# liubingqi7/audio-motion-avatar

Hardware: AMD Instinct MI355X
Metric: rendered frames/sec @512x512, 10k Gaussians (static triplane decode + SMPL-X LBS + tile rasterize) (higher is better)
Workload: dtype f32 (LBS blend-shape product: fp16 x 2 split operands with fp32 accumulation, fp32-equivalent; everything else plain fp32)

## Files before the change

### audio-motion-avatar_amd/_lib.py

```python
import ctypes
import os

_HERE = os.path.dirname(os.path.abspath(__file__))
LIB_PATH = os.environ.get("AMAV_LIB") or os.path.join(_HERE, "csrc", "libamav_hip.so")

c_float_p = ctypes.c_void_p


class AmavError(RuntimeError):
    pass


class Attr(ctypes.Structure):

    _fields_ = [("ptr", ctypes.c_void_p), ("frame_stride", ctypes.c_int64), ("elem_stride", ctypes.c_int32),
                ("_pad", ctypes.c_int32)]


class RasterArgs(ctypes.Structure):
    _fields_ = [
        ("num_frames", ctypes.c_int32), ("num_gaussians", ctypes.c_int32), ("height", ctypes.c_int32),
        ("width", ctypes.c_int32),
        ("means3d", Attr), ("rotations", Attr), ("scales", Attr), ("opacities", Attr), ("colors", Attr),
        ("viewmatrix", ctypes.c_void_p), ("projmatrix", ctypes.c_void_p), ("tanfov", ctypes.c_void_p),
# ... 81 lines not shown
    "amav_gemm_library_version": (ctypes.c_char_p, []),
    "amav_last_error": (ctypes.c_char_p, []),
    "amav_device_count": (ctypes.c_int, []),
    "amav_event_create": (ctypes.c_int, [ctypes.POINTER(ctypes.c_void_p)]),
    "amav_event_destroy": (ctypes.c_int, [ctypes.c_void_p]),
    "amav_event_record": (ctypes.c_int, [ctypes.c_void_p, ctypes.c_void_p]),
    "amav_event_elapsed_ms": (ctypes.c_int, [ctypes.c_void_p, ctypes.c_void_p, ctypes.POINTER(ctypes.c_float)]),
    "amav_camera_from_intrinsics": (ctypes.c_int, [ctypes.c_int, c_float_p, c_float_p, ctypes.c_int, ctypes.c_int,
                                                   ctypes.c_float, ctypes.c_float, c_float_p, c_float_p, c_float_p,
                                                   c_float_p, ctypes.c_void_p]),
    "amav_rasterize_workspace_bytes": (ctypes.c_size_t, [ctypes.c_int, ctypes.c_int, ctypes.c_int, ctypes.c_int,
                                                         ctypes.c_int64]),
    "amav_rasterize_forward": (ctypes.c_int, [ctypes.POINTER(RasterArgs), ctypes.c_void_p]),
    "amav_rasterize_decode_forward": (ctypes.c_int, [ctypes.POINTER(RasterArgs), ctypes.POINTER(DecodeSource),
                                                     ctypes.c_void_p]),
    "amav_rasterize_status": (ctypes.c_int, [ctypes.c_void_p, ctypes.POINTER(ctypes.c_int64),
                                             ctypes.POINTER(ctypes.c_int64), ctypes.POINTER(ctypes.c_int32),
                                             ctypes.c_void_p]),
    "amav_rasterize_backward_bytes": (ctypes.c_size_t, [ctypes.c_int, ctypes.c_int, ctypes.c_int64]),
    "amav_rasterize_backward": (ctypes.c_int, [ctypes.POINTER(RasterArgs), ctypes.POINTER(RasterBackwardArgs),
                                               ctypes.c_void_p]),
    "amav_frames_to_rgb8": (ctypes.c_int, [ctypes.c_int64, c_float_p, ctypes.c_void_p, ctypes.c_void_p]),
    "amav_add_layernorm": (ctypes.c_int, [ctypes.c_int64, ctypes.c_int, ctypes.c_int64, c_float_p, c_float_p, c_float_p,
                                          c_float_p, c_float_p, c_float_p, c_float_p, ctypes.c_float, c_float_p,
                                          ctypes.c_void_p, ctypes.c_int, ctypes.c_int, ctypes.c_void_p]),
    "amav_geglu": (ctypes.c_int, [ctypes.c_int64, ctypes.c_int, c_float_p, ctypes.c_int64, c_float_p, c_float_p,
                                  ctypes.c_void_p, ctypes.c_int, ctypes.c_void_p]),
    "amav_split_operand": (ctypes.c_int, [ctypes.c_int64, ctypes.c_int, c_float_p, ctypes.c_int64, ctypes.c_int,
                                          ctypes.c_int, ctypes.c_int, ctypes.c_void_p, ctypes.c_void_p]),
    "amav_frames_wire_bytes": (ctypes.c_size_t, [ctypes.c_int, ctypes.c_int, ctypes.c_int, ctypes.c_int64]),
# ... 137 lines not shown
```

### audio-motion-avatar_amd/csrc/amav_common.h

```cpp
#pragma once
#include <hip/hip_runtime.h>

#include <cstdarg>
#include <cstdint>
#include <cstdio>

#include "../../include/amav.h"

namespace amav {

constexpr int kWave = 64;

char *error_buffer();

inline int fail(int code, const char *fmt, ...) {
    va_list ap;
    va_start(ap, fmt);
    vsnprintf(error_buffer(), 512, fmt, ap);
    va_end(ap);
    return code;
}

#define AMAV_REQUIRE(cond, ...)                                         \
    do {                                                                \
// ... 3 lines not shown
inline int check_launch(const char *what) {
    hipError_t e = hipGetLastError();
    if (e != hipSuccess) return fail(AMAV_ERR_LAUNCH, "%s: %s", what, hipGetErrorString(e));
    return AMAV_OK;
}

inline size_t align_up(size_t v, size_t a) { return (v + a - 1) / a * a; }

constexpr int kWireHeaderInts = 16;
constexpr int kWireMagic = 0x414d4156;
constexpr int kWireTileBytes = 16 * 16 * 3;
inline size_t wire_payload_at(int F, int tiles) { return ((size_t)(kWireHeaderInts + F + tiles) * 4 + 15) / 16 * 16; }

int option_attn();
int option_lbs();

hipError_t zero_async(void *ptr, size_t bytes, hipStream_t stream);

struct Carver {
    char *base;
    size_t off = 0;
    explicit Carver(void *b) : base(static_cast<char *>(b)) {}
    template <typename T>
    T *take(size_t count) {
        off = align_up(off, 256);
        T *p = base ? reinterpret_cast<T *>(base + off) : nullptr;
        off += count * sizeof(T);
        return p;
    }
    size_t total() const { return align_up(off, 256); }
// ... 4 lines not shown
```

### audio-motion-avatar_amd/csrc/api.hip

```cpp
#include <atomic>
#include <cstdlib>
#include <cstring>

#include "amav_common.h"

namespace amav {

char *error_buffer() {
    static thread_local char buf[512] = {0};
    return buf;
}

static std::atomic<int> g_option_attn{-1}, g_option_lbs{-1};
int option_attn() { return g_option_attn.load(std::memory_order_relaxed); }
int option_lbs() { return g_option_lbs.load(std::memory_order_relaxed); }

static int clear_mode() {
    static const int mode = [] {
        const char *e = getenv("AMAV_CLEAR");
        return (e && e[0] == 'm') ? 1 : 0;
    }();
    return mode;
}

__global__ __launch_bounds__(256) void zero_words_kernel(unsigned *__restrict__ dst, size_t words) {
    const size_t i = (size_t)blockIdx.x * 256 + threadIdx.x;
    const size_t quads = words >> 2;
    if ((reinterpret_cast<uintptr_t>(dst) & 15) == 0) {
        if (i < quads) reinterpret_cast<uint4 *>(dst)[i] = make_uint4(0u, 0u, 0u, 0u);
        if (i < (words & 3)) dst[quads * 4 + i] = 0u;
// ... 104 lines not shown
extern "C" int amav_set_option(const char *name, const char *value) {
    AMAV_REQUIRE(name && value, "amav_set_option: NULL argument");
    const bool dflt = strcmp(value, "default") == 0;
    if (strcmp(name, "attn") == 0) {
        const int v = dflt ? -1 : strcmp(value, "f32") == 0 ? 0 : strcmp(value, "bf16") == 0 ? 1 : strcmp(value, "fp16") == 0 ? 2 : -2;
        AMAV_REQUIRE(v != -2, "amav_set_option: attn = \"%s\" (expected fp16, bf16, f32 or default)", value);
        amav::g_option_attn.store(v);
        return AMAV_OK;
    }
    if (strcmp(name, "lbs") == 0) {
        const int v = dflt ? -1 : strcmp(value, "f32") == 0 ? 0 : strcmp(value, "split") == 0 ? 1 : -2;
        AMAV_REQUIRE(v != -2, "amav_set_option: lbs = \"%s\" (expected split, f32 or default)", value);
        amav::g_option_lbs.store(v);
        return AMAV_OK;
    }
    return amav::fail(AMAV_ERR_INVALID_ARG, "amav_set_option: unknown option \"%s\"", name);
}
```

### audio-motion-avatar_amd/csrc/decode_quad.h

```cpp
#pragma once
#include <hip/hip_runtime.h>

namespace amav {
namespace decode {

template <int K>
__device__ __forceinline__ float quad_bcast(float v) {
    return __int_as_float(__builtin_amdgcn_mov_dpp(__float_as_int(v), K * 0x55, 0xf, 0xf, true));
}
template <int K>
__device__ __forceinline__ int quad_bcast_i(int v) {
    return __builtin_amdgcn_mov_dpp(v, K * 0x55, 0xf, 0xf, true);
}

__device__ __forceinline__ void quad_point(float v0, float v1, float v2, float &p0, float &p1, float &p2) {
#pragma clang fp contract(off)
    p0 = fmaf(quad_bcast<0>(v0) + quad_bcast<1>(v0), 0.5f, (quad_bcast<2>(v0) + quad_bcast<3>(v0)) * 0.5f) * 0.5f;
    p1 = fmaf(quad_bcast<0>(v1) + quad_bcast<1>(v1), 0.5f, (quad_bcast<2>(v1) + quad_bcast<3>(v1)) * 0.5f) * 0.5f;
    p2 = ((quad_bcast<0>(v2) + quad_bcast<1>(v2)) * 0.5f + (quad_bcast<2>(v2) + quad_bcast<3>(v2)) * 0.5f) * 0.5f;
}

__device__ __forceinline__ float clamp_unit(float p, float radius) {
#pragma clang fp contract(off)
    return fminf(fmaxf(p / radius, -1.0f), 1.0f);
}

struct PlaneTaps {
    int ix0, iy0;
    float wx0, wx1, wy0, wy1;
    int off[4];
    float w[4];
    bool in[4];
};
__device__ __forceinline__ PlaneTaps plane_taps(float gx, float gy, int R) {
#pragma clang fp contract(off)
    const float sx = fmaf(gx + 1.0f, (float)R, -1.0f), sy = fmaf(gy + 1.0f, (float)R, -1.0f);
    const float fx = floorf(sx * 0.5f), fy = floorf(sy * 0.5f);
    PlaneTaps t;
    t.ix0 = (int)fx, t.iy0 = (int)fy;
    t.wx1 = fmaf(sx, 0.5f, -fx), t.wx0 = fmaf(-sx, 0.5f, fx + 1.0f);
    t.wy1 = fmaf(sy, 0.5f, -fy), t.wy0 = fmaf(-sy, 0.5f, fy + 1.0f);
#pragma unroll
    for (int dy = 0; dy < 2; ++dy)
#pragma unroll
        for (int dx = 0; dx < 2; ++dx) {
            const int x = t.ix0 + dx, y = t.iy0 + dy;
            const bool in = x >= 0 && x < R && y >= 0 && y < R;
            const int cx = min(max(x, 0), R - 1), cy = min(max(y, 0), R - 1);
            t.in[dy * 2 + dx] = in;
            t.w[dy * 2 + dx] = in ? (dx ? t.wx1 : t.wx0) * (dy ? t.wy1 : t.wy0) : 0.0f;
            t.off[dy * 2 + dx] = (cy * R + cx) * 4;
        }
    return t;
}

struct QuadTaps {
    int off[12];
    float w[12];
};
__device__ __forceinline__ QuadTaps quad_taps(float p0, float p1, float p2, float radius, int R, int q) {
#pragma clang fp contract(off)
    const float u0 = clamp_unit(p0, radius), u1 = clamp_unit(p1, radius), u2 = clamp_unit(p2, radius);
    const PlaneTaps pt = plane_taps(q == 2 ? u1 : u0, q == 0 ? u1 : u2, R);
    QuadTaps t;
    const int RR4 = R * R * 4;
#pragma unroll
    for (int k = 0; k < 4; ++k) {
        t.w[k] = quad_bcast<0>(pt.w[k]), t.w[4 + k] = quad_bcast<1>(pt.w[k]), t.w[8 + k] = quad_bcast<2>(pt.w[k]);
        t.off[k] = quad_bcast_i<0>(pt.off[k]);
        t.off[4 + k] = RR4 + quad_bcast_i<1>(pt.off[k]);
        t.off[8 + k] = 2 * RR4 + quad_bcast_i<2>(pt.off[k]);
    }
    return t;
}

__device__ __forceinline__ float4 group_raw(const float4 (&tv)[12], const float (&tw)[12], const float4 (&wp)[4],
                                            float p0, float p1, float p2) {
#pragma clang fp contract(off)
    float4 acc = make_float4(0.f, 0.f, 0.f, 0.f);
#pragma unroll
    for (int k = 0; k < 12; ++k) {
        const float w = tw[k];
        const float4 v = tv[k];
        acc.x = fmaf(v.x, w, acc.x), acc.y = fmaf(v.y, w, acc.y), acc.z = fmaf(v.z, w, acc.z), acc.w = fmaf(v.w, w, acc.w);
    }
    const float4 w0 = wp[0], w1 = wp[1], w2 = wp[2], w3 = wp[3];
    acc.x += fmaf(w0.z, p2, fmaf(w0.y, p1, w0.x * p0)) + w0.w;
    acc.y += fmaf(w1.z, p2, fmaf(w1.x, p0, w1.y * p1)) + w1.w;
// ... 33 lines not shown
```

### audio-motion-avatar_amd/csrc/rasterizer.hip

```cpp
#include <algorithm>
#include <cmath>
#include <cstddef>
#include <cstdlib>

#include "amav_common.h"
#include "decode_quad.h"
#include "raster_project.h"
#include "raster_workspace.h"

namespace amav {
namespace raster {

#ifndef AMAV_BIN_ABLATE
#define AMAV_BIN_ABLATE 0
#endif
#ifndef AMAV_ABLATE
#define AMAV_ABLATE 0
#endif
constexpr int kRenderWavesPerSimd = 4;
constexpr int kFusedMinFrames = 96;
constexpr int kSortCap = 512;
constexpr int kBigLdsCap = 2048;
constexpr int kBigBlocks = 1280;

// ... 17 lines not shown
    float4 *geom;
    uint4 *rectd;
    int *tile_off;
    unsigned long long *keys;
    unsigned *sorted;
    int *big_list;
    int4 *queue;
    int *empty_list;
    int *slice_counts;
    Status *status;
};

static inline int bin_slices(int F) { return F >= kFusedMinFrames ? 0 : std::min(16, std::max(1, (256 + F - 1) / F)); }

static inline size_t queue_capacity(int F, int gx, int gy) { return (size_t)F * ((gy + kQueues - 1) / kQueues) * gx; }

static Buffers carve(void *ws, int F, int N, int gx, int gy, long long cap, size_t *bytes) {
    const int T = gx * gy;
    Carver c(ws);
    Buffers b;
    b.status = c.take<Status>(1);
    b.geom = c.take<float4>(((size_t)F * N + 1024) * 3);
    b.rectd = c.take<uint4>((size_t)F * N + 1024);
    b.tile_off = c.take<int>((size_t)F * (T + 1));
    b.keys = c.take<unsigned long long>((size_t)cap);
    b.sorted = c.take<unsigned>((size_t)cap);
    b.big_list = c.take<int>((size_t)F * T);
    b.queue = c.take<int4>((size_t)kQueues * kBuckets * queue_capacity(F, gx, gy));
    b.empty_list = c.take<int>((size_t)F * T);
    b.slice_counts = c.take<int>((size_t)F * bin_slices(F) * T);
// ... 21 lines not shown
    int wire_cap;
    unsigned wire_bg;
    int stash;
    int slices;
    Buffers buf;
    struct {
        const float4 *proj;
        const float *vertices;
        const int *idx4;
        const float *transl;
        const float4 *wpoint;
        float4 *out;
        float radius;
        int R, V;
        int rec_lds;
    } dec;
};

__device__ __forceinline__ int opaque(int x) {
    asm volatile("" : "+v"(x));
    return x;
}
__device__ __forceinline__ int lane_now() {
    int l;
    asm volatile("v_mbcnt_lo_u32_b32 %0, -1, 0\n\tv_mbcnt_hi_u32_b32 %0, -1, %0" : "=v"(l));
    return l;
}
__device__ __forceinline__ unsigned zero_now() {
    unsigned z;
    asm volatile("v_mov_b32 %0, 0" : "=v"(z));
// ... 178 lines not shown
    for (int o = 32; o > 0; o >>= 1) up += __shfl_xor(up, o, 64);
    if ((threadIdx.x & 63) == 0) part[threadIdx.x >> 6] = up;
    __syncthreads();
    if (threadIdx.x == 0) {
        const int sum = part[0] + part[1] + part[2] + part[3];
        if (sum) atomicAdd(reinterpret_cast<unsigned long long *>(&p.buf.status->total), (unsigned long long)sum);
    }
}

template <bool kFused, bool kPacked, bool kDecode = false>
__global__ __launch_bounds__(1024) void bin_kernel(Params p) {
    extern __shared__ int bin_lds[];
    int *counts = bin_lds;
    int *cursor = bin_lds + p.T;
    int *scratch = bin_lds + 2 * p.T + 3 * kQueues * (kBuckets + 1);
    uint2 *stash = reinterpret_cast<uint2 *>(scratch + 48);
    const int f = blockIdx.x;
#ifdef AMAV_BIN_STAMPS
#define AMAV_BIN_STAMP(k)                                                                                        \
    do {                                                                                                         \
        __syncthreads();                                                                                         \
        if (p.stamps && threadIdx.x == 0) p.stamps[(size_t)p.F * p.T * 6 + (size_t)f * 8 + (k)] = __builtin_amdgcn_s_memrealtime(); \
    } while (0)
#else
#define AMAV_BIN_STAMP(k)
#endif
    AMAV_BIN_STAMP(0);
    for (int t = threadIdx.x; t < p.T; t += blockDim.x) counts[t] = 0;
    if (kDecode && threadIdx.x < 4) scratch[40 + threadIdx.x] = 0;
    __syncthreads();

// ... 9 lines not shown
        auto project = [&](const GaussRec &rec, int i) {
            int up = 0;
            float4 g[3] = {make_float4(0.f, 0.f, 0.f, 0.f), make_float4(0.f, 0.f, 0.f, 0.f), make_float4(0.f, 0.f, 0.f, 0.f)};
            uint4 rd = preprocess_one(p, rec, cam, up, g);
            const bool real = i < p.N;
            if (!real) rd = make_uint4(0u, 0u, 0u, 0u), up = 0;
            upstream += up;
#if AMAV_BIN_ABLATE != 1
            if (rd.w) {
                const int rx0 = rd.x & 0xffff, ry0 = rd.x >> 16, rx1 = rd.y & 0xffff, ry1 = rd.y >> 16;
                for (int ty = ry0; ty < ry1; ++ty)
                    for (int tx = rx0; tx < rx1; ++tx) atomicAdd(&counts[ty * p.gx + tx], 1);
            }
#endif
            if (p.stash && real)
                stash[i] = make_uint2((rd.x & 0xff) | ((rd.x >> 16) << 8) | ((rd.y & 0xff) << 16) | ((rd.y >> 16) << 24), rd.z);
            const size_t gi = real ? (size_t)f * p.N + i : (size_t)p.F * p.N + threadIdx.x;
            if (!kDecode) p.buf.rectd[gi] = rd;
            float4 *dst = p.buf.geom + gi * 3;
            dst[0] = g[0], dst[1] = g[1], dst[2] = g[2];
        };
        if (kDecode) {
            constexpr int kRounds = 4, kSlot = kRounds * 128, kWaves = 8;
            float4 *recs = reinterpret_cast<float4 *>(reinterpret_cast<char *>(bin_lds) + p.dec.rec_lds);
            int *filled = scratch + 40, *drained = scratch + 42;
            const int N = p.N, groups = (N + kSlot - 1) / kSlot;
            bool stuck = false;
            auto wait_ge = [&](int *c, int v) {
                for (int n = 0; __hip_atomic_load(c, __ATOMIC_RELAXED, __HIP_MEMORY_SCOPE_WORKGROUP) < v; ++n) {
                    if (n > (1 << 22)) {
                        stuck = true;
                        break;
                    }
                    __builtin_amdgcn_s_sleep(1);
                }
                __builtin_amdgcn_fence(__ATOMIC_ACQUIRE, "workgroup");
            };
            auto signal = [&](int *c) {
                __builtin_amdgcn_fence(__ATOMIC_RELEASE, "workgroup");
                if ((threadIdx.x & 63) == 0) __hip_atomic_fetch_add(c, 1, __ATOMIC_RELAXED, __HIP_MEMORY_SCOPE_WORKGROUP);
            };
            if (threadIdx.x < kWaves * 64) {
                const int q = threadIdx.x & 3, slot = threadIdx.x >> 2;
                const int R = p.dec.R;
                const float4 *pl0 = p.dec.proj + (size_t)f * 3 * R * R * 4 + q;
                const float *vf = p.dec.vertices + (size_t)f * p.dec.V * 3;
                const float4 wp[4] = {p.dec.wpoint[q * 4], p.dec.wpoint[q * 4 + 1], p.dec.wpoint[q * 4 + 2], p.dec.wpoint[q * 4 + 3]};
                float tx = 0.f, ty = 0.f, tz = 0.f;
                if (p.dec.transl && q == 0) tx = p.dec.transl[f * 3], ty = p.dec.transl[f * 3 + 1], tz = p.dec.transl[f * 3 + 2];
                auto index_of = [&](int n) { return p.dec.idx4[(size_t)min(n, N - 1) * 4 + q]; };
                int idx[kRounds];
                float v[kRounds][3];
#pragma unroll
                for (int r = 0; r < kRounds; ++r) idx[r] = index_of(r * 128 + slot);
#pragma unroll
                for (int r = 0; r < kRounds; ++r) {
                    const float *vp = vf + (size_t)idx[r] * 3;
                    v[r][0] = vp[0], v[r][1] = vp[1], v[r][2] = vp[2];
                }
#pragma unroll
                for (int r = 0; r < kRounds; ++r) idx[r] = index_of(kSlot + r * 128 + slot);
                for (int k = 0; k < groups; ++k) {
                    const int s = k & 1;
                    float4 *ring = recs + s * 4 * kSlot + q * kSlot;
                    wait_ge(&drained[s], kWaves * (k >> 1));
#pragma unroll
                    for (int r = 0; r < kRounds; ++r) {
                        float p0, p1, p2;
                        decode::quad_point(v[r][0], v[r][1], v[r][2], p0, p1, p2);
                        const decode::QuadTaps t = decode::quad_taps(p0, p1, p2, p.dec.radius, R, q);
                        float4 tv[12];
#pragma unroll
                        for (int j = 0; j < 12; ++j) tv[j] = pl0[t.off[j]];
                        ring[r * 128 + slot] = decode::quad_record(tv, t.w, wp, p0, p1, p2, tx, ty, tz, q);
                    }
                    signal(&filled[s]);
#pragma unroll
                    for (int r = 0; r < kRounds; ++r) {
                        const float *vp = vf + (size_t)idx[r] * 3;
                        v[r][0] = vp[0], v[r][1] = vp[1], v[r][2] = vp[2];
                    }
#pragma unroll
                    for (int r = 0; r < kRounds; ++r) idx[r] = index_of((k + 2) * kSlot + r * 128 + slot);
                }
            } else {
                const int j = threadIdx.x - kWaves * 64;
                float4 *outf = p.dec.out + (size_t)f * N * 4;
                for (int k = 0; k < groups; ++k) {
                    const int s = k & 1;
                    const float4 *ring = recs + s * 4 * kSlot + j;
                    wait_ge(&filled[s], kWaves * ((k >> 1) + 1));
                    GaussRec rec;
                    rec.r0 = ring[0], rec.r1 = ring[kSlot], rec.r2 = ring[2 * kSlot], rec.r3 = ring[3 * kSlot];
                    signal(&drained[s]);
                    const int i = k * kSlot + j;
                    if (i < N) {
                        float4 *o = outf + (size_t)i * 4;
                        o[0] = rec.r0, o[1] = rec.r1, o[2] = rec.r2, o[3] = rec.r3;
                    }
// ... 19 lines not shown
        block_exclusive_scan(upstream, scratch, &upstream_total);
        if (threadIdx.x == 0)
            atomicAdd(reinterpret_cast<unsigned long long *>(&p.buf.status->total), (unsigned long long)upstream_total);
    } else {
        int *sc = p.buf.slice_counts + (size_t)f * p.slices * p.T;
        for (int t = threadIdx.x; t < p.T; t += blockDim.x) {
            int run = 0;
            for (int b = 0; b < p.slices; ++b) {
                const int c = sc[(size_t)b * p.T + t];
                sc[(size_t)b * p.T + t] = run;
                run += c;
            }
            counts[t] = run;
        }
    }
    __syncthreads();
    AMAV_BIN_STAMP(1);

    const int per = (p.T + (int)blockDim.x - 1) / (int)blockDim.x;
    const int t0 = threadIdx.x * per;
    int local = 0;
    for (int k = 0; k < per; ++k)
        if (t0 + k < p.T) local += counts[t0 + k];
    int total;
    int run = block_exclusive_scan(local, scratch, &total);
    int *off = p.buf.tile_off + (size_t)f * (p.T + 1);
    for (int k = 0; k < per; ++k) {
        const int t = t0 + k;
        if (t < p.T) {
            const int c = counts[t];
            cursor[t] = run;
            off[t] = run;
            run += c;
            if (c > kSortCap) {
                const int slot = atomicAdd(&p.buf.status->big_count, 1);
                p.buf.big_list[slot] = f * p.T + t;
            }
        }
    }
    const bool fits = (long long)total <= p.cap_per_frame;
// ... 1153 lines not shown
    AMAV_REQUIRE(a->num_frames > 0 && a->num_gaussians > 0 && a->height > 0 && a->width > 0,
                 "amav_rasterize_forward: bad sizes F=%d N=%d H=%d W=%d", a->num_frames, a->num_gaussians, a->height,
                 a->width);
    AMAV_REQUIRE(a->means3d.ptr && a->rotations.ptr && a->scales.ptr && a->opacities.ptr && a->colors.ptr,
                 "amav_rasterize_forward: NULL Gaussian attribute");
    AMAV_REQUIRE(a->viewmatrix && a->projmatrix && a->tanfov, "amav_rasterize_forward: NULL camera");
    AMAV_REQUIRE(a->out_rgba != nullptr, "amav_rasterize_forward: out_rgba is NULL");
    AMAV_REQUIRE(a->workspace != nullptr, "amav_rasterize_forward: workspace is NULL");
    AMAV_REQUIRE(a->instance_capacity >= 0, "amav_rasterize_forward: negative instance_capacity");
    AMAV_REQUIRE((reinterpret_cast<uintptr_t>(a->out_rgba) & 15) == 0, "amav_rasterize_forward: out_rgba not 16-B aligned");
    const int F = a->num_frames, N = a->num_gaussians;
    const int gx = (a->width + kTile - 1) / kTile, gy = (a->height + kTile - 1) / kTile;
    AMAV_REQUIRE(gx < 65536 && gy < 65536, "amav_rasterize_forward: image too large");
    const int T = gx * gy;
    AMAV_REQUIRE((long long)F * T < (1ll << 31), "amav_rasterize_forward: F * tiles overflows int32");
    const size_t bin_lds = ((size_t)2 * T + 48 + 3 * kQueues * (kBuckets + 1)) * sizeof(int);
    AMAV_REQUIRE(bin_lds <= 160 * 1024, "amav_rasterize_forward: %d tiles need %zu B of LDS in the binning block (max 160 KiB)",
                 T, bin_lds);
    const bool stash = bin_lds + 8 + (size_t)N * 8 <= 160 * 1024 && gx <= 255 && gy <= 255 && a->out_radii == nullptr;
    const size_t rec_lds = align_up(bin_lds + (size_t)N * 8, 16);
    const bool fits_decode = stash && rec_lds + 1024 * 64 <= 160 * 1024;
    const long long cap_per_frame = a->instance_capacity / F;
    AMAV_REQUIRE(cap_per_frame < (1ll << 31), "amav_rasterize_forward: per-frame instance capacity overflows int32");
    size_t need = 0;
    Params p;
    p.dec = {};
    p.buf = carve(a->workspace, F, N, gx, gy, cap_per_frame * F, &need);
    if (a->workspace_bytes < need)
        return fail(AMAV_ERR_WORKSPACE, "amav_rasterize_forward: workspace %zu < required %zu", a->workspace_bytes, need);
    p.F = F, p.N = N, p.H = a->height, p.W = a->width, p.gx = gx, p.gy = gy, p.T = T;
    p.means3d = a->means3d, p.rotations = a->rotations, p.scales = a->scales, p.opacities = a->opacities;
    p.colors = a->colors;
    p.view = a->viewmatrix, p.proj = a->projmatrix, p.tanfov = a->tanfov;
    p.bg[0] = a->bg[0], p.bg[1] = a->bg[1], p.bg[2] = a->bg[2];
    p.scale_modifier = a->scale_modifier;
    p.apply_activations = a->apply_activations;
// ... 53 lines not shown
                     "amav_rasterize_decode_forward: bad decode source (R=%d V=%d radius=%g)", d->resolution, d->num_verts,
                     (double)d->radius);
        AMAV_REQUIRE(d->proj && d->vertices && d->idx4 && d->head_w_point,
                     "amav_rasterize_decode_forward: NULL decode input");
        AMAV_REQUIRE(((reinterpret_cast<uintptr_t>(d->proj) | reinterpret_cast<uintptr_t>(d->idx4) |
                       reinterpret_cast<uintptr_t>(d->head_w_point)) & 15) == 0,
                     "amav_rasterize_decode_forward: proj/idx4/head_w_point not 16-B aligned");
        p.dec.proj = reinterpret_cast<const float4 *>(d->proj);
        p.dec.vertices = d->vertices;
        p.dec.idx4 = d->idx4;
        p.dec.transl = d->transl;
        p.dec.wpoint = reinterpret_cast<const float4 *>(d->head_w_point);
        p.dec.out = reinterpret_cast<float4 *>(const_cast<float *>(b0));
        p.dec.radius = d->radius;
        p.dec.R = d->resolution, p.dec.V = d->num_verts;
        p.dec.rec_lds = (int)rec_lds;
        if (!decode_fused) {
            const int rc = amav_triplane_sample_decode_indexed(F, N, d->resolution, d->num_verts, d->proj, d->vertices,
                                                               d->idx4, d->transl, d->radius, d->head_w_point,
                                                               const_cast<float *>(b0), stream);
            if (rc != AMAV_OK) return rc;
        }
    }
    if (zero_async(p.buf.status, sizeof(Status), stream) != hipSuccess)
        return fail(AMAV_ERR_LAUNCH, "amav_rasterize_forward: status clear failed");
    if (p.wire_header && zero_async(p.wire_header, (size_t)kWireHeaderInts * 4, stream) != hipSuccess)
        return fail(AMAV_ERR_LAUNCH, "amav_rasterize_forward: wire header clear failed");

    if (F < kFusedMinFrames && F <= 65535) {
        const dim3 pre_grid((unsigned)((N + 255) / 256), (unsigned)F);
        if (packed)
            preprocess_kernel<true><<<pre_grid, 256, 0, stream>>>(p);
        else
            preprocess_kernel<false><<<pre_grid, 256, 0, stream>>>(p);
        const dim3 slice_grid((unsigned)p.slices, (unsigned)F);
        slice_count_kernel<<<slice_grid, 1024, (size_t)T * sizeof(int), stream>>>(p);
        bin_kernel<false, false><<<F, 1024, bin_lds, stream>>>(p);
        slice_scatter_kernel<<<slice_grid, 1024, (size_t)T * sizeof(int), stream>>>(p);
    } else if (decode_fused)
        bin_kernel<true, true, true><<<F, 1024, rec_lds + 1024 * 64, stream>>>(p);
    else if (packed)
        bin_kernel<true, true><<<F, 1024, bin_lds + (stash ? 8 + (size_t)N * 8 : 0), stream>>>(p);
    else
        bin_kernel<true, false><<<F, 1024, bin_lds + (stash ? 8 + (size_t)N * 8 : 0), stream>>>(p);
    sort_big_kernel<<<kBigBlocks, 256, 0, stream>>>(p);
    const unsigned blocks = render_grid(a->out_inv_depth != nullptr);
    if (a->profile_start_event) (void)hipEventRecord(static_cast<hipEvent_t>(a->profile_start_event), stream);
    if (a->out_inv_depth)
        render_kernel<true><<<blocks, 64, 0, stream>>>(p);
    else
        render_kernel<false><<<blocks, 64, 0, stream>>>(p);
    if (a->profile_stop_event) (void)hipEventRecord(static_cast<hipEvent_t>(a->profile_stop_event), stream);
    return check_launch("amav_rasterize_forward");
}

extern "C" int amav_rasterize_forward(const amav_raster_args *a, void *stream) { return rasterize_forward(a, nullptr, stream); }

extern "C" int amav_rasterize_decode_forward(const amav_raster_args *a, const amav_decode_source *d, void *stream) {
    AMAV_REQUIRE(d != nullptr, "amav_rasterize_decode_forward: decode source is NULL");
    return rasterize_forward(a, d, stream);
}

namespace amav {
namespace raster {
__global__ __launch_bounds__(256) void tile_counts_kernel(int F, int T, const Status *__restrict__ st,
                                                          const int *__restrict__ tile_off, int *__restrict__ out) {
    const int i = blockIdx.x * blockDim.x + threadIdx.x;
    if (i >= F * T) return;
    const int f = i / T, t = i - f * T;
    const int *off = tile_off + (size_t)f * (T + 1);
// ... 45 lines not shown
```

### audio-motion-avatar_amd/csrc/triplane.hip

```cpp
#include <cstdlib>

#include "amav_common.h"
#include "decode_quad.h"
#include "triplane_region.h"

namespace amav {
namespace triplane {

typedef float f32x4 __attribute__((ext_vector_type(4)));

template <int kUnroll, bool kNT>
__global__ __launch_bounds__(256) void project_kernel(int C, int RR, const float *__restrict__ tokens,
                                                      long long frame_stride, const float *__restrict__ wplane,
                                                      float *__restrict__ out, const float *__restrict__ boxes,
                                                      float radius, int R) {
    extern __shared__ __align__(16) float w_lds[];
    const int bx = blockIdx.z;
    int q = bx * blockDim.x + threadIdx.x;
    const int plane = blockIdx.x, f = blockIdx.y;
    if (boxes) {
        const TexelRect rc = region_of(boxes + (size_t)f * 6, plane, radius, R);
        const int c0 = rc.x0 >> 2, per_row = (rc.x1 >> 2) - c0 + 1, rows = rc.y1 - rc.y0 + 1;
        if (bx * (int)blockDim.x >= per_row * rows) return;
        const int row = q / per_row;
// ... 197 lines not shown
        float acc = 0.0f;
#pragma unroll
        for (int q = 0; q < 4; ++q)
            if (off[q] >= 0) acc += img[off[q]] * wt[q];
        tile[k * 65 + lane] = acc;
    }
    __syncthreads();
    for (int p = wave; p < 64; p += 4) {
        if (n0 + p < N) out[((size_t)f * N + n0 + p) * 3 * C + oc0 + lane] = tile[lane * 65 + p];
    }
}

__global__ __launch_bounds__(1024) void bbox_kernel(int N, const float *__restrict__ points, float *__restrict__ boxes) {
    __shared__ float part[16][7];
    const int f = blockIdx.x;
    const float *pp = points + (size_t)f * N * 3;
    const int total = 3 * N;
    float lo[3] = {__builtin_inff(), __builtin_inff(), __builtin_inff()};
    float hi[3] = {-__builtin_inff(), -__builtin_inff(), -__builtin_inff()};
    float bad = 0.f;
    for (int e0 = threadIdx.x * 3; e0 < total; e0 += blockDim.x * 3) {
#pragma unroll
        for (int d = 0; d < 3; ++d) {
            const float v = pp[e0 + d];
            lo[d] = fminf(lo[d], v), hi[d] = fmaxf(hi[d], v);
            if (v != v) bad = 1.f;
        }
    }
#pragma unroll
    for (int o = 32; o > 0; o >>= 1) {
#pragma unroll
        for (int d = 0; d < 3; ++d) {
            lo[d] = fminf(lo[d], __shfl_xor(lo[d], o, 64));
            hi[d] = fmaxf(hi[d], __shfl_xor(hi[d], o, 64));
        }
        bad = fmaxf(bad, __shfl_xor(bad, o, 64));
    }
    const int wave = threadIdx.x >> 6, nwaves = blockDim.x >> 6;
    if ((threadIdx.x & 63) == 0) {
#pragma unroll
        for (int d = 0; d < 3; ++d) part[wave][d] = lo[d], part[wave][3 + d] = hi[d];
        part[wave][6] = bad;
    }
    __syncthreads();
    if (threadIdx.x < 6) {
        const int d = threadIdx.x;
        float any_bad = 0.f, v = part[0][d];
        for (int w = 0; w < nwaves; ++w) {
            any_bad += part[w][6];
            v = d < 3 ? fminf(v, part[w][d]) : fmaxf(v, part[w][d]);
        }
        if (any_bad > 0.f) v = d < 3 ? -__builtin_inff() : __builtin_inff();
        boxes[(size_t)f * 6 + d] = v;
    }
}

}
}

using namespace amav;
using namespace amav::triplane;

extern "C" int amav_points_bbox(int F, int N, const float *points, float *out_boxes, void *stream) {
    AMAV_REQUIRE(F > 0 && N > 0 && points && out_boxes, "amav_points_bbox: bad sizes F=%d N=%d or NULL pointer", F, N);
    bbox_kernel<<<F, 1024, 0, static_cast<hipStream_t>(stream)>>>(N, points, out_boxes);
    return check_launch("amav_points_bbox");
}

extern "C" int amav_triplane_project(int F, int C, int R, const float *tokens, int64_t frame_stride,
// ... 88 lines not shown
```

### audio-motion-avatar_amd/csrc/triplane_region.h

```cpp
#pragma once
#include <hip/hip_runtime.h>

namespace amav {
namespace triplane {

struct TexelRect {
    int x0, x1, y0, y1;
};
__device__ __forceinline__ int tap_floor(float p, float radius, int R) {
    const float u = fminf(fmaxf(p / radius, -1.0f), 1.0f);
    return (int)floorf(((u + 1.0f) * (float)R - 1.0f) * 0.5f);
}
__device__ __forceinline__ TexelRect region_of(const float *__restrict__ box, int plane, float radius, int R) {
    const int ax = plane == 2 ? 1 : 0, ay = plane == 0 ? 1 : 2;
    TexelRect r;
    r.x0 = min(max(tap_floor(box[ax], radius, R), 0), R - 1);
    r.x1 = min(max(tap_floor(box[3 + ax], radius, R) + 1, 0), R - 1);
    r.y0 = min(max(tap_floor(box[ay], radius, R), 0), R - 1);
    r.y1 = min(max(tap_floor(box[3 + ay], radius, R) + 1, 0), R - 1);
    return r;
}

}
}
```

### audio-motion-avatar_amd/ops.py

```python
import ctypes
import os

import torch

from . import _lib
from ._lib import (AmavError, Attr, BodyTables, DecodeSource, LbsBackwardArgs, PoseParts, RasterArgs,
                   RasterBackwardArgs, TriplaneDecodeBackwardArgs, check)

SCALE_BIAS = 3.9
OPACITY_BIAS = 0.0
SCALE_MAX = 0.1
GAUSS_STRIDE = 16
REC_XYZ, REC_OPACITY, REC_ROT, REC_SCALE, REC_COLOR = 0, 3, 4, 8, 12


def tensor_version(t: torch.Tensor) -> int:
    return -1 if t.is_inference() else t._version


def set_option(name: str, value: str):
    check(_lib.lib().amav_set_option(name.encode(), value.encode()), "amav_set_option")


def _stream():
    return ctypes.c_void_p(torch.cuda.current_stream().cuda_stream)


def _need(t: torch.Tensor, name: str, dtype=torch.float32):
    if not isinstance(t, torch.Tensor):
        raise AmavError(f"{name}: expected a torch.Tensor, got {type(t).__name__}")
    if not t.is_cuda:
        raise AmavError(f"{name}: tensor is on {t.device}; this package only runs on an MI355X (HIP) device")
    if t.dtype != dtype:
        raise AmavError(f"{name}: dtype {t.dtype}, expected {dtype}")
    return t

# ... 1373 lines not shown
```

### include/amav.h

```cpp
#ifndef AMAV_H
#define AMAV_H

#include <stddef.h>
#include <stdint.h>

#ifdef __cplusplus
extern "C" {
#endif

#define AMAV_OK 0
#define AMAV_ERR_INVALID_ARG (-1)
#define AMAV_ERR_LAUNCH (-2)
#define AMAV_ERR_WORKSPACE (-3)
#define AMAV_ERR_NO_DEVICE (-4)

#define AMAV_TILE 16
#define AMAV_GAUSS_STRIDE 16

const char *amav_version(void);
const char *amav_last_error(void);
int amav_device_count(void);
int amav_set_option(const char *name, const char *value);

int amav_event_create(void **event);
// ... 61 lines not shown
    float *debug_alpha;
} amav_raster_backward_args;
size_t amav_rasterize_backward_bytes(int num_frames, int num_gaussians, int64_t max_frame_instances);
int amav_rasterize_backward(const amav_raster_args *fwd, const amav_raster_backward_args *bwd, void *stream);

typedef struct amav_decode_source {
    int32_t resolution, num_verts;
    const float *proj;
    const float *vertices;
    const int32_t *idx4;
    const float *transl;
    float radius;
    const float *head_w_point;
} amav_decode_source;
int amav_rasterize_decode_forward(const amav_raster_args *args, const amav_decode_source *src, void *stream);

int amav_frames_to_rgb8(int64_t num_pixels, const float *rgba_dev, uint8_t *out_rgb8_dev, void *stream);

int amav_rasterize_tile_counts(const void *workspace, int num_frames, int num_gaussians, int height, int width,
                               int64_t instance_capacity, int32_t *out_counts_dev, void *stream);
size_t amav_frames_wire_bytes(int num_frames, int height, int width, int64_t capacity_tiles);
int amav_frames_pack_tiles(int num_frames, int height, int width, const float *rgba_dev, const float *background_host3,
                           const int32_t *tile_hint_dev, int64_t capacity_tiles, void *wire_dev, size_t wire_bytes,
                           void *stream);
int amav_frames_unpack_tiles(int num_buffers, int num_frames, int height, int width, int64_t capacity_tiles,
                             const void *wire_all_dev, size_t wire_stride, uint8_t *out_rgb8_dev, int32_t *status_dev,
                             void *stream);
int amav_frames_unpack_tiles_delta(int num_buffers, int num_frames, int height, int width, int64_t capacity_tiles,
                                   const void *wire_all_dev, size_t wire_stride, uint8_t *out_rgb8_dev,
                                   int32_t *tile_state_dev, int32_t *status_dev, void *stream);
// ... 199 lines not shown
```

Baseline: 321,500.

## Stage triplane texel region into LDS for fused decode-bin kernel

In the fused decode+bin kernel, each frame's vertex bounding box is computed in-block and mapped to texel rectangles on the three planes. When those fit in the spare LDS, the rectangles are copied into shared memory and bilinear taps read from LDS instead of global memory. To free LDS, the per-gaussian stash is written to global memory first and reloaded into LDS after binning. This adds a bbox reduction, extra barriers and a full 160 KiB LDS allocation per block, which may cut occupancy, and can be turned off with the decode_taps=global option.

```diff
diff --git a/audio-motion-avatar_amd/_lib.py b/audio-motion-avatar_amd/_lib.py
--- a/audio-motion-avatar_amd/_lib.py
+++ b/audio-motion-avatar_amd/_lib.py
@@ -119,6 +119,7 @@
     "amav_rasterize_forward": (ctypes.c_int, [ctypes.POINTER(RasterArgs), ctypes.c_void_p]),
     "amav_rasterize_decode_forward": (ctypes.c_int, [ctypes.POINTER(RasterArgs), ctypes.POINTER(DecodeSource),
                                                      ctypes.c_void_p]),
+    "amav_decode_bin_region_texels": (ctypes.c_int, [ctypes.c_int, ctypes.c_int, ctypes.c_int]),
     "amav_rasterize_status": (ctypes.c_int, [ctypes.c_void_p, ctypes.POINTER(ctypes.c_int64),
                                              ctypes.POINTER(ctypes.c_int64), ctypes.POINTER(ctypes.c_int32),
                                              ctypes.c_void_p]),
diff --git a/audio-motion-avatar_amd/csrc/amav_common.h b/audio-motion-avatar_amd/csrc/amav_common.h
--- a/audio-motion-avatar_amd/csrc/amav_common.h
+++ b/audio-motion-avatar_amd/csrc/amav_common.h
@@ -41,6 +41,7 @@
 
 int option_attn();
 int option_lbs();
+int option_decode_taps();
 
 hipError_t zero_async(void *ptr, size_t bytes, hipStream_t stream);
 
diff --git a/audio-motion-avatar_amd/csrc/api.hip b/audio-motion-avatar_amd/csrc/api.hip
--- a/audio-motion-avatar_amd/csrc/api.hip
+++ b/audio-motion-avatar_amd/csrc/api.hip
@@ -11,9 +11,10 @@
     return buf;
 }
 
-static std::atomic<int> g_option_attn{-1}, g_option_lbs{-1};
+static std::atomic<int> g_option_attn{-1}, g_option_lbs{-1}, g_option_decode_taps{-1};
 int option_attn() { return g_option_attn.load(std::memory_order_relaxed); }
 int option_lbs() { return g_option_lbs.load(std::memory_order_relaxed); }
+int option_decode_taps() { return g_option_decode_taps.load(std::memory_order_relaxed); }
 
 static int clear_mode() {
     static const int mode = [] {
@@ -148,5 +149,11 @@
         amav::g_option_lbs.store(v);
         return AMAV_OK;
     }
+    if (strcmp(name, "decode_taps") == 0) {
+        const int v = dflt ? -1 : strcmp(value, "global") == 0 ? 0 : strcmp(value, "lds") == 0 ? 1 : -2;
+        AMAV_REQUIRE(v != -2, "amav_set_option: decode_taps = \"%s\" (expected lds, global or default)", value);
+        amav::g_option_decode_taps.store(v);
+        return AMAV_OK;
+    }
     return amav::fail(AMAV_ERR_INVALID_ARG, "amav_set_option: unknown option \"%s\"", name);
 }
diff --git a/audio-motion-avatar_amd/csrc/decode_quad.h b/audio-motion-avatar_amd/csrc/decode_quad.h
--- a/audio-motion-avatar_amd/csrc/decode_quad.h
+++ b/audio-motion-avatar_amd/csrc/decode_quad.h
@@ -32,7 +32,7 @@
     float w[4];
     bool in[4];
 };
-__device__ __forceinline__ PlaneTaps plane_taps(float gx, float gy, int R) {
+__device__ __forceinline__ PlaneTaps plane_taps(float gx, float gy, int R, int pitch, int base) {
 #pragma clang fp contract(off)
     const float sx = fmaf(gx + 1.0f, (float)R, -1.0f), sy = fmaf(gy + 1.0f, (float)R, -1.0f);
     const float fx = floorf(sx * 0.5f), fy = floorf(sy * 0.5f);
@@ -49,29 +49,32 @@
             const int cx = min(max(x, 0), R - 1), cy = min(max(y, 0), R - 1);
             t.in[dy * 2 + dx] = in;
             t.w[dy * 2 + dx] = in ? (dx ? t.wx1 : t.wx0) * (dy ? t.wy1 : t.wy0) : 0.0f;
-            t.off[dy * 2 + dx] = (cy * R + cx) * 4;
+            t.off[dy * 2 + dx] = base + (cy * pitch + cx) * 4;
         }
     return t;
 }
+__device__ __forceinline__ PlaneTaps plane_taps(float gx, float gy, int R) { return plane_taps(gx, gy, R, R, 0); }
 
 struct QuadTaps {
     int off[12];
     float w[12];
 };
-__device__ __forceinline__ QuadTaps quad_taps(float p0, float p1, float p2, float radius, int R, int q) {
+__device__ __forceinline__ QuadTaps quad_taps(float p0, float p1, float p2, float radius, int R, int q, int pitch, int base) {
 #pragma clang fp contract(off)
     const float u0 = clamp_unit(p0, radius), u1 = clamp_unit(p1, radius), u2 = clamp_unit(p2, radius);
-    const PlaneTaps pt = plane_taps(q == 2 ? u1 : u0, q == 0 ? u1 : u2, R);
+    const PlaneTaps pt = plane_taps(q == 2 ? u1 : u0, q == 0 ? u1 : u2, R, pitch, base);
     QuadTaps t;
-    const int RR4 = R * R * 4;
 #pragma unroll
     for (int k = 0; k < 4; ++k) {
         t.w[k] = quad_bcast<0>(pt.w[k]), t.w[4 + k] = quad_bcast<1>(pt.w[k]), t.w[8 + k] = quad_bcast<2>(pt.w[k]);
         t.off[k] = quad_bcast_i<0>(pt.off[k]);
-        t.off[4 + k] = RR4 + quad_bcast_i<1>(pt.off[k]);
-        t.off[8 + k] = 2 * RR4 + quad_bcast_i<2>(pt.off[k]);
+        t.off[4 + k] = quad_bcast_i<1>(pt.off[k]);
+        t.off[8 + k] = quad_bcast_i<2>(pt.off[k]);
     }
     return t;
+}
+__device__ __forceinline__ QuadTaps quad_taps(float p0, float p1, float p2, float radius, int R, int q) {
+    return quad_taps(p0, p1, p2, radius, R, q, R, q * R * R * 4);
 }
 
 __device__ __forceinline__ float4 group_raw(const float4 (&tv)[12], const float (&tw)[12], const float4 (&wp)[4],
diff --git a/audio-motion-avatar_amd/csrc/rasterizer.hip b/audio-motion-avatar_amd/csrc/rasterizer.hip
--- a/audio-motion-avatar_amd/csrc/rasterizer.hip
+++ b/audio-motion-avatar_amd/csrc/rasterizer.hip
@@ -7,6 +7,7 @@
 #include "decode_quad.h"
 #include "raster_project.h"
 #include "raster_workspace.h"
+#include "triplane_region.h"
 
 namespace amav {
 namespace raster {
@@ -55,6 +56,24 @@
 static inline int bin_slices(int F) { return F >= kFusedMinFrames ? 0 : std::min(16, std::max(1, (256 + F - 1) / F)); }
 
 static inline size_t queue_capacity(int F, int gx, int gy) { return (size_t)F * ((gy + kQueues - 1) / kQueues) * gx; }
+
+constexpr size_t kLdsBytes = 160 * 1024, kRingBytes = 1024 * 64, kTexelBytes = 64;
+struct DecodeLds {
+    size_t counters;
+    bool stash, fits;
+    size_t ring_at, region_at;
+    int region_texels;
+};
+static DecodeLds decode_lds(int N, int gx, int gy, bool radii) {
+    DecodeLds l;
+    l.counters = ((size_t)2 * gx * gy + 48 + 3 * kQueues * (kBuckets + 1)) * sizeof(int);
+    l.stash = l.counters + 8 + (size_t)N * 8 <= kLdsBytes && gx <= 255 && gy <= 255 && !radii;
+    l.fits = l.stash && align_up(l.counters + (size_t)N * 8, 16) + kRingBytes <= kLdsBytes;
+    l.ring_at = align_up(l.counters, 16);
+    l.region_at = l.ring_at + kRingBytes;
+    l.region_texels = l.fits ? (int)((kLdsBytes - l.region_at) / kTexelBytes) : 0;
+    return l;
+}
 
 static Buffers carve(void *ws, int F, int N, int gx, int gy, long long cap, size_t *bytes) {
     const int T = gx * gy;
@@ -106,6 +125,8 @@
         float radius;
         int R, V;
         int rec_lds;
+        int region_lds;
+        int region_cap;
     } dec;
 };
 
@@ -314,7 +335,9 @@
     int *counts = bin_lds;
     int *cursor = bin_lds + p.T;
     int *scratch = bin_lds + 2 * p.T + 3 * kQueues * (kBuckets + 1);
-    uint2 *stash = reinterpret_cast<uint2 *>(scratch + 48);
+    uint2 *stash = kDecode ? reinterpret_cast<uint2 *>(reinterpret_cast<char *>(bin_lds) + p.dec.rec_lds)
+                           : reinterpret_cast<uint2 *>(scratch + 48);
+    uint2 *stash_mem = reinterpret_cast<uint2 *>(p.buf.rectd + (size_t)blockIdx.x * p.N);
     const int f = blockIdx.x;
 #ifdef AMAV_BIN_STAMPS
 #define AMAV_BIN_STAMP(k)                                                                                        \
@@ -354,7 +377,8 @@
             }
 #endif
             if (p.stash && real)
-                stash[i] = make_uint2((rd.x & 0xff) | ((rd.x >> 16) << 8) | ((rd.y & 0xff) << 16) | ((rd.y >> 16) << 24), rd.z);
+                (kDecode ? stash_mem : stash)[i] =
+                    make_uint2((rd.x & 0xff) | ((rd.x >> 16) << 8) | ((rd.y & 0xff) << 16) | ((rd.y >> 16) << 24), rd.z);
             const size_t gi = real ? (size_t)f * p.N + i : (size_t)p.F * p.N + threadIdx.x;
             if (!kDecode) p.buf.rectd[gi] = rd;
             float4 *dst = p.buf.geom + gi * 3;
@@ -380,19 +404,26 @@
                 __builtin_amdgcn_fence(__ATOMIC_RELEASE, "workgroup");
                 if ((threadIdx.x & 63) == 0) __hip_atomic_fetch_add(c, 1, __ATOMIC_RELAXED, __HIP_MEMORY_SCOPE_WORKGROUP);
             };
-            if (threadIdx.x < kWaves * 64) {
-                const int q = threadIdx.x & 3, slot = threadIdx.x >> 2;
-                const int R = p.dec.R;
-                const float4 *pl0 = p.dec.proj + (size_t)f * 3 * R * R * 4 + q;
-                const float *vf = p.dec.vertices + (size_t)f * p.dec.V * 3;
-                const float4 wp[4] = {p.dec.wpoint[q * 4], p.dec.wpoint[q * 4 + 1], p.dec.wpoint[q * 4 + 2], p.dec.wpoint[q * 4 + 3]};
-                float tx = 0.f, ty = 0.f, tz = 0.f;
+            const bool decoder = threadIdx.x < kWaves * 64;
+            const int q = threadIdx.x & 3, slot = threadIdx.x >> 2;
+            const int R = p.dec.R;
+            const float4 *pl0 = p.dec.proj + (size_t)f * 3 * R * R * 4 + q;
+            const float *vf = p.dec.vertices + (size_t)f * p.dec.V * 3;
+            auto index_of = [&](int n) { return p.dec.idx4[(size_t)min(n, N - 1) * 4 + q]; };
+            int idx[kRounds] = {0, 0, 0, 0};
+            float v[kRounds][3] = {};
+            float4 wp0 = make_float4(0.f, 0.f, 0.f, 0.f), wp1 = wp0, wp2 = wp0, wp3 = wp0;
+            float tx = 0.f, ty = 0.f, tz = 0.f;
+            if (decoder) {
+#pragma unroll
+                for (int r = 0; r < kRounds; ++r) idx[r] = index_of(r * 128 + slot);
+                wp0 = p.dec.wpoint[q * 4], wp1 = p.dec.wpoint[q * 4 + 1], wp2 = p.dec.wpoint[q * 4 + 2], wp3 = p.dec.wpoint[q * 4 + 3];
                 if (p.dec.transl && q == 0) tx = p.dec.transl[f * 3], ty = p.dec.transl[f * 3 + 1], tz = p.dec.transl[f * 3 + 2];
-                auto index_of = [&](int n) { return p.dec.idx4[(size_t)min(n, N - 1) * 4 + q]; };
-                int idx[kRounds];
-                float v[kRounds][3];
-#pragma unroll
-                for (int r = 0; r < kRounds; ++r) idx[r] = index_of(r * 128 + slot);
+            }
+            int region_pitch = 0, region_base = 0;
+            float(*part)[7] = reinterpret_cast<float(*)[7]>(recs);
+            if (p.dec.region_cap) triplane::box_partials(vf, p.dec.V, part);
+            if (decoder) {
 #pragma unroll
                 for (int r = 0; r < kRounds; ++r) {
                     const float *vp = vf + (size_t)idx[r] * 3;
@@ -400,29 +431,77 @@
                 }
 #pragma unroll
                 for (int r = 0; r < kRounds; ++r) idx[r] = index_of(kSlot + r * 128 + slot);
-                for (int k = 0; k < groups; ++k) {
-                    const int s = k & 1;
-                    float4 *ring = recs + s * 4 * kSlot + q * kSlot;
-                    wait_ge(&drained[s], kWaves * (k >> 1));
-#pragma unroll
-                    for (int r = 0; r < kRounds; ++r) {
-                        float p0, p1, p2;
-                        decode::quad_point(v[r][0], v[r][1], v[r][2], p0, p1, p2);
-                        const decode::QuadTaps t = decode::quad_taps(p0, p1, p2, p.dec.radius, R, q);
-                        float4 tv[12];
-#pragma unroll
-                        for (int j = 0; j < 12; ++j) tv[j] = pl0[t.off[j]];
-                        ring[r * 128 + slot] = decode::quad_record(tv, t.w, wp, p0, p1, p2, tx, ty, tz, q);
+            }
+            if (p.dec.region_cap) {
+                __syncthreads();
+                float *shared_box = &part[16][0];
+                if (threadIdx.x < 6) shared_box[threadIdx.x] = triplane::box_component(part, (int)(blockDim.x >> 6), (int)threadIdx.x);
+                __syncthreads();
+                float box[6];
+#pragma unroll
+                for (int d = 0; d < 6; ++d) box[d] = shared_box[d];
+                const triplane::TexelRect ra = triplane::region_of(box, 0, p.dec.radius, R);
+                const triplane::TexelRect rb = triplane::region_of(box, 1, p.dec.radius, R);
+                const triplane::TexelRect rc = triplane::region_of(box, 2, p.dec.radius, R);
+                const int wa = ra.x1 - ra.x0 + 1, wb = rb.x1 - rb.x0 + 1, wc = rc.x1 - rc.x0 + 1;
+                const int fb = wa * (ra.y1 - ra.y0 + 1), fc = fb + wb * (rb.y1 - rb.y0 + 1);
+                const int texels = fc + wc * (rc.y1 - rc.y0 + 1);
+                if (texels <= p.dec.region_cap && (R & (R - 1)) == 0) {
+                    constexpr int kPer = (int)(((kLdsBytes - kRingBytes) / 16 + 1023) / 1024);
+                    float4 *region = reinterpret_cast<float4 *>(reinterpret_cast<char *>(bin_lds) + p.dec.region_lds);
+                    const float4 *src = p.dec.proj + (size_t)f * 3 * R * R * 4;
+                    float4 held[kPer];
+#pragma unroll
+                    for (int k = 0; k < kPer; ++k) {
+                        const int e = min((int)threadIdx.x + k * 1024, texels * 4 - 1), t = e >> 2;
+                        const bool in_b = t >= fb && t < fc, in_c = t >= fc;
+                        const int w = in_c ? wc : in_b ? wb : wa, local = t - (in_c ? fc : in_b ? fb : 0);
+                        const int x0 = in_c ? rc.x0 : in_b ? rb.x0 : ra.x0, y0 = in_c ? rc.y0 : in_b ? rb.y0 : ra.y0;
+                        const int row = local / w, col = local - row * w;
+                        held[k] = src[(((in_c ? 2 : in_b ? 1 : 0) * R + y0 + row) * R + x0 + col) * 4 + (e & 3)];
                     }
-                    signal(&filled[s]);
-#pragma unroll
-                    for (int r = 0; r < kRounds; ++r) {
-                        const float *vp = vf + (size_t)idx[r] * 3;
-                        v[r][0] = vp[0], v[r][1] = vp[1], v[r][2] = vp[2];
+#pragma unroll
+                    for (int k = 0; k < kPer; ++k)
+                        if ((int)threadIdx.x + k * 1024 < texels * 4) region[threadIdx.x + k * 1024] = held[k];
+                    region_pitch = q == 0 ? wa : q == 1 ? wb : q == 2 ? wc : 1;
+                    region_base = q == 0 ? -(ra.y0 * wa + ra.x0) * 4 : q == 1 ? (fb - (rb.y0 * wb + rb.x0)) * 4
+                                                                              : (fc - (rc.y0 * wc + rc.x0)) * 4;
+                }
+            }
+            __syncthreads();
+            AMAV_BIN_STAMP(5);
+            if (decoder) {
+                const float4 wp[4] = {wp0, wp1, wp2, wp3};
+                auto decode_groups = [&](auto *texels, int pitch, int base) {
+                    for (int k = 0; k < groups; ++k) {
+                        const int s = k & 1;
+                        float4 *ring = recs + s * 4 * kSlot + q * kSlot;
+                        wait_ge(&drained[s], kWaves * (k >> 1));
+#pragma unroll
+                        for (int r = 0; r < kRounds; ++r) {
+                            float p0, p1, p2;
+                            decode::quad_point(v[r][0], v[r][1], v[r][2], p0, p1, p2);
+                            const decode::QuadTaps t = decode::quad_taps(p0, p1, p2, p.dec.radius, R, q, pitch, base);
+                            float4 tv[12];
+#pragma unroll
+                            for (int j = 0; j < 12; ++j) tv[j] = texels[t.off[j]];
+                            ring[r * 128 + slot] = decode::quad_record(tv, t.w, wp, p0, p1, p2, tx, ty, tz, q);
+                        }
+                        signal(&filled[s]);
+#pragma unroll
+                        for (int r = 0; r < kRounds; ++r) {
+                            const float *vp = vf + (size_t)idx[r] * 3;
+                            v[r][0] = vp[0], v[r][1] = vp[1], v[r][2] = vp[2];
+                        }
+#pragma unroll
+                        for (int r = 0; r < kRounds; ++r) idx[r] = index_of((k + 2) * kSlot + r * 128 + slot);
                     }
-#pragma unroll
-                    for (int r = 0; r < kRounds; ++r) idx[r] = index_of((k + 2) * kSlot + r * 128 + slot);
-                }
+                };
+                if (region_pitch)
+                    decode_groups(reinterpret_cast<const float4 *>(reinterpret_cast<char *>(bin_lds) + p.dec.region_lds) + q,
+                                  region_pitch, region_base);
+                else
+                    decode_groups(pl0, R, q * R * R * 4);
             } else {
                 const int j = threadIdx.x - kWaves * 64;
                 float4 *outf = p.dec.out + (size_t)f * N * 4;
@@ -472,8 +551,16 @@
             counts[t] = run;
         }
     }
+    if (kDecode) __builtin_amdgcn_fence(__ATOMIC_RELEASE, "workgroup");
     __syncthreads();
     AMAV_BIN_STAMP(1);
+    constexpr int kStashPer = 12;
+    uint2 held[kStashPer];
+    if (kDecode) {
+        __builtin_amdgcn_fence(__ATOMIC_ACQUIRE, "workgroup");
+#pragma unroll
+        for (int k = 0; k < kStashPer; ++k) held[k] = stash_mem[min((int)threadIdx.x + k * 1024, p.N - 1)];
+    }
 
     const int per = (p.T + (int)blockDim.x - 1) / (int)blockDim.x;
     const int t0 = threadIdx.x * per;
@@ -482,6 +569,11 @@
         if (t0 + k < p.T) local += counts[t0 + k];
     int total;
     int run = block_exclusive_scan(local, scratch, &total);
+    if (kDecode) {
+#pragma unroll
+        for (int k = 0; k < kStashPer; ++k)
+            if ((int)threadIdx.x + k * 1024 < p.N) stash[threadIdx.x + k * 1024] = held[k];
+    }
     int *off = p.buf.tile_off + (size_t)f * (p.T + 1);
     for (int k = 0; k < per; ++k) {
         const int t = t0 + k;
@@ -1665,12 +1757,11 @@
     AMAV_REQUIRE(gx < 65536 && gy < 65536, "amav_rasterize_forward: image too large");
     const int T = gx * gy;
     AMAV_REQUIRE((long long)F * T < (1ll << 31), "amav_rasterize_forward: F * tiles overflows int32");
-    const size_t bin_lds = ((size_t)2 * T + 48 + 3 * kQueues * (kBuckets + 1)) * sizeof(int);
+    const DecodeLds dl = decode_lds(N, gx, gy, a->out_radii != nullptr);
+    const size_t bin_lds = dl.counters;
     AMAV_REQUIRE(bin_lds <= 160 * 1024, "amav_rasterize_forward: %d tiles need %zu B of LDS in the binning block (max 160 KiB)",
                  T, bin_lds);
-    const bool stash = bin_lds + 8 + (size_t)N * 8 <= 160 * 1024 && gx <= 255 && gy <= 255 && a->out_radii == nullptr;
-    const size_t rec_lds = align_up(bin_lds + (size_t)N * 8, 16);
-    const bool fits_decode = stash && rec_lds + 1024 * 64 <= 160 * 1024;
+    const bool stash = dl.stash, fits_decode = dl.fits;
     const long long cap_per_frame = a->instance_capacity / F;
     AMAV_REQUIRE(cap_per_frame < (1ll << 31), "amav_rasterize_forward: per-frame instance capacity overflows int32");
     size_t need = 0;
@@ -1754,7 +1845,8 @@
         p.dec.out = reinterpret_cast<float4 *>(const_cast<float *>(b0));
         p.dec.radius = d->radius;
         p.dec.R = d->resolution, p.dec.V = d->num_verts;
-        p.dec.rec_lds = (int)rec_lds;
+        p.dec.rec_lds = (int)dl.ring_at, p.dec.region_lds = (int)dl.region_at;
+        p.dec.region_cap = option_decode_taps() == 0 ? 0 : dl.region_texels;
         if (!decode_fused) {
             const int rc = amav_triplane_sample_decode_indexed(F, N, d->resolution, d->num_verts, d->proj, d->vertices,
                                                                d->idx4, d->transl, d->radius, d->head_w_point,
@@ -1778,7 +1870,7 @@
         bin_kernel<false, false><<<F, 1024, bin_lds, stream>>>(p);
         slice_scatter_kernel<<<slice_grid, 1024, (size_t)T * sizeof(int), stream>>>(p);
     } else if (decode_fused)
-        bin_kernel<true, true, true><<<F, 1024, rec_lds + 1024 * 64, stream>>>(p);
+        bin_kernel<true, true, true><<<F, 1024, kLdsBytes, stream>>>(p);
     else if (packed)
         bin_kernel<true, true><<<F, 1024, bin_lds + (stash ? 8 + (size_t)N * 8 : 0), stream>>>(p);
     else
@@ -1794,6 +1886,13 @@
     return check_launch("amav_rasterize_forward");
 }
 
+extern "C" int amav_decode_bin_region_texels(int num_gaussians, int height, int width) {
+    if (num_gaussians <= 0 || height <= 0 || width <= 0) return 0;
+    const int gx = (width + kTile - 1) / kTile, gy = (height + kTile - 1) / kTile;
+    if (gx >= 65536 || gy >= 65536) return 0;
+    return decode_lds(num_gaussians, gx, gy, false).region_texels;
+}
+
 extern "C" int amav_rasterize_forward(const amav_raster_args *a, void *stream) { return rasterize_forward(a, nullptr, stream); }
 
 extern "C" int amav_rasterize_decode_forward(const amav_raster_args *a, const amav_decode_source *d, void *stream) {
diff --git a/audio-motion-avatar_amd/csrc/triplane.hip b/audio-motion-avatar_amd/csrc/triplane.hip
--- a/audio-motion-avatar_amd/csrc/triplane.hip
+++ b/audio-motion-avatar_amd/csrc/triplane.hip
@@ -235,45 +235,9 @@
 __global__ __launch_bounds__(1024) void bbox_kernel(int N, const float *__restrict__ points, float *__restrict__ boxes) {
     __shared__ float part[16][7];
     const int f = blockIdx.x;
-    const float *pp = points + (size_t)f * N * 3;
-    const int total = 3 * N;
-    float lo[3] = {__builtin_inff(), __builtin_inff(), __builtin_inff()};
-    float hi[3] = {-__builtin_inff(), -__builtin_inff(), -__builtin_inff()};
-    float bad = 0.f;
-    for (int e0 = threadIdx.x * 3; e0 < total; e0 += blockDim.x * 3) {
-#pragma unroll
-        for (int d = 0; d < 3; ++d) {
-            const float v = pp[e0 + d];
-            lo[d] = fminf(lo[d], v), hi[d] = fmaxf(hi[d], v);
-            if (v != v) bad = 1.f;
-        }
-    }
-#pragma unroll
-    for (int o = 32; o > 0; o >>= 1) {
-#pragma unroll
-        for (int d = 0; d < 3; ++d) {
-            lo[d] = fminf(lo[d], __shfl_xor(lo[d], o, 64));
-            hi[d] = fmaxf(hi[d], __shfl_xor(hi[d], o, 64));
-        }
-        bad = fmaxf(bad, __shfl_xor(bad, o, 64));
-    }
-    const int wave = threadIdx.x >> 6, nwaves = blockDim.x >> 6;
-    if ((threadIdx.x & 63) == 0) {
-#pragma unroll
-        for (int d = 0; d < 3; ++d) part[wave][d] = lo[d], part[wave][3 + d] = hi[d];
-        part[wave][6] = bad;
-    }
+    box_partials(points + (size_t)f * N * 3, N, part);
     __syncthreads();
-    if (threadIdx.x < 6) {
-        const int d = threadIdx.x;
-        float any_bad = 0.f, v = part[0][d];
-        for (int w = 0; w < nwaves; ++w) {
-            any_bad += part[w][6];
-            v = d < 3 ? fminf(v, part[w][d]) : fmaxf(v, part[w][d]);
-        }
-        if (any_bad > 0.f) v = d < 3 ? -__builtin_inff() : __builtin_inff();
-        boxes[(size_t)f * 6 + d] = v;
-    }
+    if (threadIdx.x < 6) boxes[(size_t)f * 6 + threadIdx.x] = box_component(part, (int)(blockDim.x >> 6), (int)threadIdx.x);
 }
 
 }
diff --git a/audio-motion-avatar_amd/csrc/triplane_region.h b/audio-motion-avatar_amd/csrc/triplane_region.h
--- a/audio-motion-avatar_amd/csrc/triplane_region.h
+++ b/audio-motion-avatar_amd/csrc/triplane_region.h
@@ -21,5 +21,54 @@
     return r;
 }
 
+
+__device__ __forceinline__ void box_partials(const float *__restrict__ pp, int N, float (*part)[7]) {
+    const int total = 3 * N, stride = (int)blockDim.x * 3;
+    float lo[3] = {__builtin_inff(), __builtin_inff(), __builtin_inff()};
+    float hi[3] = {-__builtin_inff(), -__builtin_inff(), -__builtin_inff()};
+    float bad = 0.f;
+    constexpr int kTrips = 12;
+    for (int e0 = threadIdx.x * 3; e0 < total; e0 += kTrips * stride) {
+        float v[kTrips][3];
+#pragma unroll
+        for (int u = 0; u < kTrips; ++u) {
+            const int e = min(e0 + u * stride, total - 3);
+#pragma unroll
+            for (int d = 0; d < 3; ++d) v[u][d] = pp[e + d];
+        }
+#pragma unroll
+        for (int u = 0; u < kTrips; ++u)
+#pragma unroll
+            for (int d = 0; d < 3; ++d) {
+                lo[d] = fminf(lo[d], v[u][d]), hi[d] = fmaxf(hi[d], v[u][d]);
+                if (v[u][d] != v[u][d]) bad = 1.f;
+            }
+    }
+#pragma unroll
+    for (int o = 32; o > 0; o >>= 1) {
+#pragma unroll
+        for (int d = 0; d < 3; ++d) {
+            lo[d] = fminf(lo[d], __shfl_xor(lo[d], o, 64));
+            hi[d] = fmaxf(hi[d], __shfl_xor(hi[d], o, 64));
+        }
+        bad = fmaxf(bad, __shfl_xor(bad, o, 64));
+    }
+    if ((threadIdx.x & 63) == 0) {
+        const int wave = threadIdx.x >> 6;
+#pragma unroll
+        for (int d = 0; d < 3; ++d) part[wave][d] = lo[d], part[wave][3 + d] = hi[d];
+        part[wave][6] = bad;
+    }
+}
+__device__ __forceinline__ float box_component(const float (*part)[7], int nwaves, int d) {
+    float any_bad = 0.f, v = part[0][d];
+    for (int w = 0; w < nwaves; ++w) {
+        any_bad += part[w][6];
+        v = d < 3 ? fminf(v, part[w][d]) : fmaxf(v, part[w][d]);
+    }
+    if (any_bad > 0.f) v = d < 3 ? -__builtin_inff() : __builtin_inff();
+    return v;
+}
+
 }
 }
diff --git a/audio-motion-avatar_amd/ops.py b/audio-motion-avatar_amd/ops.py
--- a/audio-motion-avatar_amd/ops.py
+++ b/audio-motion-avatar_amd/ops.py
@@ -20,6 +20,10 @@
 
 def set_option(name: str, value: str):
     check(_lib.lib().amav_set_option(name.encode(), value.encode()), "amav_set_option")
+
+
+def decode_bin_region_texels(num_gaussians: int, height: int, width: int) -> int:
+    return int(_lib.lib().amav_decode_bin_region_texels(int(num_gaussians), int(height), int(width)))
 
 
 def _stream():
diff --git a/include/amav.h b/include/amav.h
--- a/include/amav.h
+++ b/include/amav.h
@@ -99,6 +99,7 @@
     const float *head_w_point;
 } amav_decode_source;
 int amav_rasterize_decode_forward(const amav_raster_args *args, const amav_decode_source *src, void *stream);
+int amav_decode_bin_region_texels(int num_gaussians, int height, int width);
 
 int amav_frames_to_rgb8(int64_t num_pixels, const float *rgba_dev, uint8_t *out_rgb8_dev, void *stream);
 
```

Measured after the change: 321,400, median of 2. About the same (-0.0%).
